# elrodrigues/deneva-plus

Measured on AMD Instinct MI355X. Metric: committed txns/sec (node) YCSB zipf0.9 at 1/2/4/8 GPUs; abort-set bit-exact, higher is better.
Workload: dtype u64; 1 GPU; YCSB config D: 16,777,216 rows/partition, 1,048,576-txn epoch in total; cc_alg=NO_WAIT, rows_per_partition=16777216, txns_per_epoch=1048576, txns_per_epoch_per_gpu=1048576, req_per_query=10, parallelism=1 GPU, decision_lanes=4, sequence_order=one origin

## Files before the change

### deneva-plus_amd/csrc/dvcc_kernels.hip

```cpp
#include <hip/hip_ext.h>

#include "dvcc_common.h"
#include "dvcc_tpcc.h"

#ifndef DVCC_PROBE_HIST_WAVES
#define DVCC_PROBE_HIST_WAVES 6
#endif

namespace dvcc {


constexpr int kPV = 4;
template <bool HIST, bool RSV>
__device__ __forceinline__ void probe_body(const Tables &tabs, const uint64_t *__restrict__ keys,
                                           const uint32_t *__restrict__ keys32,
                                                  const uint8_t *__restrict__ types,
                                                  const uint32_t *__restrict__ acc_txn,
                                                  const uint8_t *__restrict__ tables, uint64_t n,
                                                  uint32_t n_txn, uint32_t slog,
                                                  uint64_t *__restrict__ pairs,
                                                  uint32_t *__restrict__ tb_start,
                                                  uint32_t *__restrict__ tb_end,
                                                  uint8_t *__restrict__ tlen,
                                                  uint32_t *__restrict__ acc_row, Counters *ctr,
// ... 334 lines not shown
                pairs[a0 + pos] = pair_pack(row, t, (pos >> slog) ? 0u : pos, wr);
            }
        }
    }
    if (bad) set_err(ctr, ERRB_TXN);
    if (big_seen) set_err(ctr, ERRB_BIG);
    if (ts_bad) set_err(ctr, ERRB_TS);
}

void launch_probe_tb(hipStream_t s, const Tables &tabs, const uint64_t *keys, const uint8_t *types,
                     const uint32_t *recs, const uint32_t *txn_begin, uint64_t n_acc, uint32_t n_txn, uint32_t K,
                     uint32_t slog, uint64_t *pairs, uint8_t *tlen, uint32_t *acc_row, Counters *ctr,
                     const uint64_t *ts, hipEvent_t ev0, hipEvent_t ev1, const uint32_t *n_acc_dev) {
#ifndef DVCC_PROBE_TB_GRID
#define DVCC_PROBE_TB_GRID 4096
#endif
    uint32_t g = (n_txn + kBlock - 1) / kBlock;
    g = g < 1 ? 1 : (g > DVCC_PROBE_TB_GRID ? DVCC_PROBE_TB_GRID : g);
    DV_LAUNCH_EV(k_probe_tb, g, kBlock, 0, s, ev0, ev1, tabs, keys, types, recs, txn_begin, n_acc, n_txn, K, slog,
                 pairs, tlen, acc_row, ctr, ts, n_acc_dev);
}


__device__ __forceinline__ uint64_t sort_n(uint64_t n, const uint32_t *n_dev) {
    return n_dev && (uint64_t)*n_dev < n ? (uint64_t)*n_dev : n;
}

__device__ __forceinline__ uint32_t row_hash(uint64_t key, uint32_t hmul, int hbits) {
    return ((uint32_t)(key >> 32) * hmul) & ((1u << hbits) - 1u);
}
template <int W>
__device__ __forceinline__ uint32_t key_digit(uint64_t key, int shift, uint32_t hmul, int hbits) {
    return hmul ? row_hash(key, hmul, hbits) >> (hbits - W) : (uint32_t)(key >> shift) & ((1u << W) - 1u);
}

__global__ __launch_bounds__(kBlock) void k_radix_hist(const uint64_t *__restrict__ in, uint64_t n,
                                                       int shift, uint32_t *__restrict__ counts,
                                                       uint32_t nblocks, const uint32_t *__restrict__ n_dev,
                                                       uint32_t hmul, int hbits) {
    __shared__ uint32_t wc[4][kRadix];
    n = sort_n(n, n_dev);
    if ((uint64_t)blockIdx.x * kTile >= n) return;
    const uint32_t tid = threadIdx.x, lane = tid & 63, wave = tid >> 6;
    for (uint32_t d = tid; d < 4 * kRadix; d += kBlock) (&wc[0][0])[d] = 0;
    __syncthreads();
    const uint64_t base = (uint64_t)blockIdx.x * kTile + wave * (64 * kIPT);
    uint64_t k[kIPT];
#pragma unroll
    for (int j = 0; j < kIPT; j++) {
        const uint64_t idx = base + j * 64 + lane;
        k[j] = idx < n ? in[idx] : 0;
    }
#pragma unroll
    for (int j = 0; j < kIPT; j++) {
        const uint64_t idx = base + j * 64 + lane;
        const bool valid = idx < n;
        const uint32_t d = key_digit<kRadixBits>(k[j], shift, hmul, hbits);
        const uint32_t d0 = __builtin_amdgcn_readfirstlane(d);
        const uint64_t vmask = __ballot(valid);
        if (__ballot(valid && d == d0) == vmask) {
            if (lane == 0) wc[wave][d0] += (uint32_t)__popcll(vmask);
        } else if (valid) {
            atomicAdd(&wc[wave][d], 1u);
        }
    }
    __syncthreads();
    for (uint32_t d = tid; d < kRadix; d += kBlock)
        counts[(uint64_t)d * nblocks + blockIdx.x] = wc[0][d] + wc[1][d] + wc[2][d] + wc[3][d];
}

__global__ __launch_bounds__(kBlock) void k_radix_scan(uint32_t *__restrict__ counts, uint32_t nblocks,
                                                       uint32_t *__restrict__ digit_tot,
                                                       const uint32_t *__restrict__ n_dev) {
    __shared__ uint32_t lds4[4];
    uint32_t *c = counts + (uint64_t)blockIdx.x * nblocks;
    if (n_dev && nblocks_for(*n_dev) < nblocks) nblocks = nblocks_for(*n_dev);
    const uint32_t tot = block_chunk_scan256(c, nblocks, lds4);
    if (threadIdx.x == 0) digit_tot[blockIdx.x] = tot;
}

__global__ __launch_bounds__(kBlock) void k_radix_scatter(
    const uint64_t *__restrict__ in, uint64_t *__restrict__ out, uint64_t n, int shift, const uint32_t *__restrict__ counts,
    const uint32_t *__restrict__ digit_tot, uint32_t nblocks, const uint32_t *__restrict__ n_dev,
    uint32_t hmul, int hbits) {
    __shared__ __attribute__((aligned(16))) uint64_t skeys[kTile];
    n = sort_n(n, n_dev);
    if ((uint64_t)blockIdx.x * kTile >= n) return;
    __shared__ uint32_t wc[4][kRadix];
    __shared__ uint32_t dstart[kRadix];
    __shared__ uint64_t gbase[kRadix];
    __shared__ uint32_t lds4[4];
    const uint32_t tid = threadIdx.x, lane = tid & 63, wave = tid >> 6;
    const uint64_t tile0 = (uint64_t)blockIdx.x * kTile;

    {
        const uint32_t d = tid;
        const uint32_t dex = block_excl_scan256(digit_tot[d], lds4, nullptr);
        gbase[d] = (uint64_t)dex + counts[(uint64_t)d * nblocks + blockIdx.x];
        for (int w = 0; w < 4; w++) wc[w][d] = 0;
    }
    __syncthreads();

    const uint64_t base = tile0 + wave * (64 * kIPT);
    uint64_t k[kIPT];
    uint32_t r[kIPT];
#pragma unroll
    for (int j = 0; j < kIPT; j++) {
        const uint64_t idx = base + j * 64 + lane;
        k[j] = idx < n ? in[idx] : 0;
    }
#pragma unroll
    for (int j = 0; j < kIPT; j++) {
        const uint64_t idx = base + j * 64 + lane;
        const bool valid = idx < n;
        const uint32_t d = key_digit<kRadixBits>(k[j], shift, hmul, hbits);
        const uint64_t vmask = __ballot(valid);
        const uint64_t peers = match_digit(d, vmask);
        const uint32_t before = wc[wave][d];
        r[j] = before + mask_rank(peers);
        if (valid && lane == (uint32_t)__builtin_ctzll(peers)) wc[wave][d] = before + (uint32_t)__popcll(peers);
    }
    __syncthreads();
    {
        const uint32_t d = tid;
        const uint32_t c0 = wc[0][d], c1 = wc[1][d], c2 = wc[2][d], c3 = wc[3][d];
        wc[0][d] = 0;
        wc[1][d] = c0;
        wc[2][d] = c0 + c1;
        wc[3][d] = c0 + c1 + c2;
        const uint32_t ds = block_excl_scan256(c0 + c1 + c2 + c3, lds4, nullptr);
        dstart[d] = ds;
        gbase[d] -= ds;
    }
    __syncthreads();
#pragma unroll
    for (int j = 0; j < kIPT; j++) {
        const uint64_t idx = base + j * 64 + lane;
        if (idx < n) {
            const uint32_t d = key_digit<kRadixBits>(k[j], shift, hmul, hbits);
            const uint32_t pos = dstart[d] + wc[wave][d] + r[j];
            skeys[pos] = k[j];
        }
    }
    __syncthreads();
    const uint32_t tile_n = (uint32_t)((n - tile0) < (uint64_t)kTile ? (n - tile0) : kTile);
    for (uint32_t p = tid; p < tile_n; p += kBlock) {
        const uint64_t key = skeys[p];
        const uint32_t d = key_digit<kRadixBits>(key, shift, hmul, hbits);
        const uint64_t dst = gbase[d] + p;
        out[dst] = key;
    }
}

template <int W>
__global__ __launch_bounds__(kBlock) void k_radix_hist_w(const uint64_t *__restrict__ in, uint64_t n, int shift,
                                                         uint32_t *__restrict__ counts, uint32_t nblocks,
                                                         const uint32_t *__restrict__ n_dev, uint32_t hmul,
                                                         int hbits) {
    constexpr uint32_t R = 1u << W;
    __shared__ uint32_t wc[4][R];
    n = sort_n(n, n_dev);
    if ((uint64_t)blockIdx.x * kTile >= n) return;
    const uint32_t tid = threadIdx.x, lane = tid & 63, wave = tid >> 6;
    for (uint32_t d = tid; d < 4 * R; d += kBlock) (&wc[0][0])[d] = 0;
    __syncthreads();
    const uint64_t base = (uint64_t)blockIdx.x * kTile + wave * (64 * kIPT);
    uint64_t k[kIPT];
#pragma unroll
    for (int j = 0; j < kIPT; j++) {
        const uint64_t idx = base + j * 64 + lane;
        k[j] = idx < n ? in[idx] : 0;
    }
#pragma unroll
    for (int j = 0; j < kIPT; j++) {
        const uint64_t idx = base + j * 64 + lane;
        const bool valid = idx < n;
        const uint32_t d = key_digit<W>(k[j], shift, hmul, hbits);
        const uint32_t d0 = __builtin_amdgcn_readfirstlane(d);
        const uint64_t vmask = __ballot(valid);
        if (__ballot(valid && d == d0) == vmask) {
            if (lane == 0) wc[wave][d0] += (uint32_t)__popcll(vmask);
        } else if (valid) {
            atomicAdd(&wc[wave][d], 1u);
        }
    }
    __syncthreads();
    for (uint32_t d = tid; d < R; d += kBlock)
        counts[(uint64_t)d * nblocks + blockIdx.x] = wc[0][d] + wc[1][d] + wc[2][d] + wc[3][d];
}

template <int W>
__global__ __launch_bounds__(kBlock) void k_radix_scatter_w(const uint64_t *__restrict__ in, uint64_t *__restrict__ out,
                                                            uint64_t n, int shift, const uint32_t *__restrict__ counts,
                                                            const uint32_t *__restrict__ digit_tot, uint32_t nblocks,
                                                            const uint32_t *__restrict__ n_dev, uint32_t hmul,
                                                            int hbits) {
    constexpr uint32_t R = 1u << W, PER = R / kBlock;
    __shared__ __attribute__((aligned(16))) uint64_t skeys[kTile];
    __shared__ uint32_t wc[4][R];
    __shared__ uint32_t dstart[R];
    __shared__ uint32_t gbase[R];
    __shared__ uint32_t lds4[4];
    n = sort_n(n, n_dev);
    if ((uint64_t)blockIdx.x * kTile >= n) return;
    const uint32_t tid = threadIdx.x, lane = tid & 63, wave = tid >> 6;
    const uint64_t tile0 = (uint64_t)blockIdx.x * kTile;
    {
        uint32_t t[PER], sum = 0;
#pragma unroll
        for (uint32_t q = 0; q < PER; q++) {
            t[q] = digit_tot[tid * PER + q];
            sum += t[q];
        }
        uint32_t pre = block_excl_scan256(sum, lds4, nullptr);
#pragma unroll
        for (uint32_t q = 0; q < PER; q++) {
            const uint32_t d = tid * PER + q;
            gbase[d] = pre + counts[(uint64_t)d * nblocks + blockIdx.x];
            pre += t[q];
            wc[0][d] = wc[1][d] = wc[2][d] = wc[3][d] = 0;
        }
    }
    __syncthreads();
    const uint64_t base = tile0 + wave * (64 * kIPT);
    uint64_t k[kIPT];
    uint32_t r[kIPT];
#pragma unroll
    for (int j = 0; j < kIPT; j++) {
        const uint64_t idx = base + j * 64 + lane;
        k[j] = idx < n ? in[idx] : 0;
    }
#pragma unroll
    for (int j = 0; j < kIPT; j++) {
        const uint64_t idx = base + j * 64 + lane;
        const bool valid = idx < n;
        const uint32_t d = key_digit<W>(k[j], shift, hmul, hbits);
        uint64_t peers = __ballot(valid);
#pragma unroll
        for (int b = 0; b < W; b++) {
            const uint32_t bit = (d >> b) & 1u;
            const uint64_t m = __ballot(bit);
            peers &= bit ? m : ~m;
        }
        const uint32_t before = wc[wave][d];
        r[j] = before + mask_rank(peers);
        if (valid && lane == (uint32_t)__builtin_ctzll(peers)) wc[wave][d] = before + (uint32_t)__popcll(peers);
    }
    __syncthreads();
    {
        uint32_t tot[PER], sum = 0;
#pragma unroll
        for (uint32_t q = 0; q < PER; q++) {
            const uint32_t d = tid * PER + q;
            const uint32_t c0 = wc[0][d], c1 = wc[1][d], c2 = wc[2][d], c3 = wc[3][d];
            wc[0][d] = 0;
            wc[1][d] = c0;
            wc[2][d] = c0 + c1;
            wc[3][d] = c0 + c1 + c2;
            tot[q] = c0 + c1 + c2 + c3;
            sum += tot[q];
        }
        uint32_t ds = block_excl_scan256(sum, lds4, nullptr);
#pragma unroll
        for (uint32_t q = 0; q < PER; q++) {
            const uint32_t d = tid * PER + q;
            dstart[d] = ds;
            gbase[d] -= ds;
            ds += tot[q];
        }
    }
    __syncthreads();
#pragma unroll
    for (int j = 0; j < kIPT; j++) {
        const uint64_t idx = base + j * 64 + lane;
        if (idx < n) {
            const uint32_t d = key_digit<W>(k[j], shift, hmul, hbits);
            skeys[dstart[d] + wc[wave][d] + r[j]] = k[j];
        }
    }
    __syncthreads();
    const uint32_t tile_n = (uint32_t)((n - tile0) < (uint64_t)kTile ? (n - tile0) : kTile);
    for (uint32_t p = tid; p < tile_n; p += kBlock) {
        const uint64_t key = skeys[p];
        const uint32_t d = key_digit<W>(key, shift, hmul, hbits);
        out[(uint64_t)gbase[d] + p] = key;
    }
}

template <int W>
void wide_pass(hipStream_t s, const uint64_t *in, uint64_t *out, uint64_t n, int shift, uint32_t *counts,
               uint32_t *digit_tot, uint32_t nb, const uint32_t *n_dev, hipEvent_t e0, hipEvent_t e1,
               uint32_t hmul = 0, int hbits = 0) {
    DV_LAUNCH((k_radix_hist_w<W>), nb, kBlock, 0, s, in, n, shift, counts, nb, n_dev, hmul, hbits);
    DV_LAUNCH(k_radix_scan, 1u << W, kBlock, 0, s, counts, nb, digit_tot, n_dev);
    DV_LAUNCH_EV((k_radix_scatter_w<W>), nb, kBlock, 0, s, e0, e1, in, out, n, shift,
                          (const uint32_t *)counts, (const uint32_t *)digit_tot, nb, n_dev, hmul, hbits);
}

constexpr int kBucketThreads = 1024;
constexpr int kBucketWaves = kBucketThreads / 64;
constexpr int kBucketIdxBits = 32 - kBucketHiMax;
constexpr uint32_t kBucketCap = 1u << kBucketIdxBits;
constexpr int kBucketSteps = (int)kBucketCap / kBucketThreads;
static_assert((2 * kBucketCap + (kBucketWaves + 2) * kRadix + kBucketWaves) * sizeof(uint32_t) <= 160u * 1024u,
              "k_bucket_sort's LDS exceeds gfx950's 160 KiB per workgroup");

__device__ __forceinline__ uint32_t bucket_rank(uint32_t d, bool valid, uint32_t *wcw, uint32_t lane) {
    const uint64_t peers = match_digit(d, __ballot(valid));
    const uint32_t before = wcw[d];
    if (valid && lane == (uint32_t)__builtin_ctzll(peers)) wcw[d] = before + (uint32_t)__popcll(peers);
    return before + mask_rank(peers);
}

__device__ __forceinline__ void bucket_bases(uint32_t (*wc)[kRadix], uint32_t *tot, uint32_t *run) {
    const uint32_t tid = threadIdx.x, lane = tid & 63;
    uint32_t sum = 0;
    if (tid < (uint32_t)kRadix) {
#pragma unroll
        for (int w = 0; w < kBucketWaves; w++) {
            const uint32_t c = wc[w][tid];
            wc[w][tid] = sum;
            sum += c;
        }
        if (!run) tot[tid] = sum;
    }
    __syncthreads();
    if (!run && tid < 64) {
        uint32_t v[4], s4 = 0;
#pragma unroll
        for (int q = 0; q < 4; q++) {
            v[q] = tot[4 * lane + q];
            s4 += v[q];
        }
        uint32_t pre = wave_incl_sum(s4, lane) - s4;
#pragma unroll
        for (int q = 0; q < 4; q++) {
            tot[4 * lane + q] = pre;
            pre += v[q];
        }
    }
    if (!run) __syncthreads();
    if (tid < (uint32_t)kRadix) {
        const uint32_t b = run ? run[tid] : tot[tid];
        if (run) run[tid] = b + sum;
#pragma unroll
        for (int w = 0; w < kBucketWaves; w++) wc[w][tid] += b;
    }
    __syncthreads();
}

#ifdef DVCC_BUCKET_STAMPS
__device__ unsigned long long g_bucket_stamps[1024 * 4];
__device__ unsigned long long g_bucket_launch[4];
__device__ unsigned long long g_bucket_lmax;
struct BucketStamp {
    uint64_t t0;
    __device__ BucketStamp() : t0(wall_clock64()) {}
    __device__ void done(uint32_t b, uint32_t m) {
        __syncthreads();
        if (threadIdx.x != 0) return;
        const unsigned long long dt = wall_clock64() - t0;
        unsigned long long *w = g_bucket_stamps + (size_t)b * 4;
        atomicAdd(w + 0, 1ull);
        atomicAdd(w + 1, dt);
        atomicAdd(w + 2, (unsigned long long)m);
        atomicMax(w + 3, dt);
        atomicMax(&g_bucket_lmax, (dt << 20) | m);
        __threadfence();
        if (atomicAdd(&g_bucket_launch[3], 1ull) == (unsigned long long)gridDim.x - 1) {
            __threadfence();
            const unsigned long long mx = atomicExch(&g_bucket_lmax, 0ull);
            atomicAdd(&g_bucket_launch[0], 1ull);
            atomicAdd(&g_bucket_launch[1], mx >> 20);
            atomicAdd(&g_bucket_launch[2], mx & 0xFFFFFull);
            g_bucket_launch[3] = 0;
        }
    }
};
extern "C" int dv_debug_bucket_stamps(uint64_t *out, uint64_t *launch) {
    if (!out || !launch) return DV_ERR_ARG;
    if (hipDeviceSynchronize() != hipSuccess) return DV_ERR_HIP;
    if (hipMemcpyFromSymbol(out, HIP_SYMBOL(g_bucket_stamps), 1024 * 4 * 8) != hipSuccess) return DV_ERR_HIP;
    if (hipMemcpyFromSymbol(launch, HIP_SYMBOL(g_bucket_launch), 4 * 8) != hipSuccess) return DV_ERR_HIP;
    static const unsigned long long zero[1024 * 4] = {};
    if (hipMemcpyToSymbol(HIP_SYMBOL(g_bucket_stamps), zero, sizeof(zero)) != hipSuccess) return DV_ERR_HIP;
    if (hipMemcpyToSymbol(HIP_SYMBOL(g_bucket_launch), zero, 4 * 8) != hipSuccess) return DV_ERR_HIP;
    return DV_OK;
}
#endif

__global__ __launch_bounds__(kBucketThreads) void k_bucket_sort(uint64_t *__restrict__ in, uint64_t *__restrict__ out,
                                                                const uint32_t *__restrict__ digit_tot,
                                                                uint32_t hmul, int hbits, int hi_bits) {
#ifdef DVCC_BUCKET_STAMPS
    BucketStamp stamp_;
    struct StampAtExit {
        BucketStamp &s;
        uint32_t b, m;
        __device__ ~StampAtExit() { s.done(b, m); }
    } stamp_exit_{stamp_, blockIdx.x, 0u};
#endif
    __shared__ uint32_t tg[2][kBucketCap];
    __shared__ uint32_t wc[kBucketWaves][kRadix];
    __shared__ uint32_t tot[kRadix], run[kRadix];
    __shared__ uint32_t s_part[kBucketWaves];
    const uint32_t tid = threadIdx.x, lane = tid & 63, wave = tid >> 6, b = blockIdx.x;
    {
        uint32_t v = tid < b ? digit_tot[tid] : 0u;
#pragma unroll
        for (int off = 32; off > 0; off >>= 1) v += __shfl_xor(v, off, 64);
        if (lane == 0) s_part[wave] = v;
    }
    __syncthreads();
    uint32_t base = 0;
#pragma unroll
    for (int w = 0; w < kBucketWaves; w++) base += s_part[w];
    const uint32_t m = digit_tot[b];
#ifdef DVCC_BUCKET_STAMPS
    stamp_exit_.m = m;
#endif
    if (m <= 1) {
        if (m == 1 && tid == 0) out[base] = in[base];
        return;
    }
    const int passes = (hi_bits + kRadixBits - 1) / kRadixBits;
    const uint32_t hmask = (1u << hi_bits) - 1u;
    if (m <= kBucketCap) {
        {
            uint64_t kv[kBucketSteps];
#pragma unroll
            for (int s = 0; s < kBucketSteps; s++) {
                const uint32_t i = s * kBucketThreads + tid;
                kv[s] = i < m ? in[base + i] : 0ull;
            }
#pragma unroll
            for (int s = 0; s < kBucketSteps; s++) {
                const uint32_t i = s * kBucketThreads + tid;
                if (i < m) tg[0][i] = ((row_hash(kv[s], hmul, hbits) & hmask) << kBucketIdxBits) | i;
            }
        }
        __syncthreads();
        const uint32_t steps = (m + kBucketThreads - 1) / kBucketThreads;
        int cur = 0;
        for (int p = 0; p < passes; p++) {
            const int sh = kBucketIdxBits + kRadixBits * p;
            for (uint32_t d = lane; d < (uint32_t)kRadix; d += 64) wc[wave][d] = 0;
            uint32_t t[kBucketSteps], r[kBucketSteps];
#pragma unroll
            for (int s = 0; s < kBucketSteps; s++) {
                if ((uint32_t)s < steps) {
                    const uint32_t e = (wave * steps + s) * 64 + lane;
                    const bool valid = e < m;
                    t[s] = valid ? tg[cur][e] : 0u;
                    r[s] = bucket_rank((t[s] >> sh) & (kRadix - 1), valid, wc[wave], lane);
                }
            }
            __syncthreads();
            bucket_bases(wc, tot, nullptr);
#pragma unroll
            for (int s = 0; s < kBucketSteps; s++) {
                if ((uint32_t)s < steps) {
                    const uint32_t e = (wave * steps + s) * 64 + lane;
                    if (e < m) tg[cur ^ 1][wc[wave][(t[s] >> sh) & (kRadix - 1)] + r[s]] = t[s];
                }
            }
            __syncthreads();
            cur ^= 1;
        }
        uint64_t kv[kBucketSteps];
#pragma unroll
        for (int s = 0; s < kBucketSteps; s++) {
            const uint32_t i = s * kBucketThreads + tid;
            kv[s] = i < m ? in[base + (tg[cur][i] & (kBucketCap - 1))] : 0ull;
        }
#pragma unroll
        for (int s = 0; s < kBucketSteps; s++) {
            const uint32_t i = s * kBucketThreads + tid;
            if (i < m) out[base + i] = kv[s];
        }
        return;
    }
    uint64_t *A = in + base, *B = out + base;
    for (int p = 0; p < passes; p++) {
        const uint64_t *src = (p & 1) ? B : A;
        uint64_t *dst = (p & 1) ? A : B;
        const int sh = kRadixBits * p;
        if (tid < (uint32_t)kRadix) tot[tid] = 0;
        __syncthreads();
        for (uint32_t i0 = 0; i0 < m; i0 += kBucketThreads) {
            const uint32_t i = i0 + tid;
            const bool valid = i < m;
            const uint32_t d = valid ? ((row_hash(src[i], hmul, hbits) & hmask) >> sh) & (kRadix - 1) : 0u;
            const uint32_t d0 = __builtin_amdgcn_readfirstlane(d);
            const uint64_t vm = __ballot(valid);
            if (__ballot(valid && d == d0) == vm) {
                if (lane == 0 && vm) atomicAdd(&tot[d0], (uint32_t)__popcll(vm));
            } else if (valid) {
                atomicAdd(&tot[d], 1u);
            }
        }
        __syncthreads();
        if (tid < 64) {
            uint32_t v[4], s4 = 0;
#pragma unroll
            for (int q = 0; q < 4; q++) {
                v[q] = tot[4 * lane + q];
                s4 += v[q];
            }
            uint32_t pre = wave_incl_sum(s4, lane) - s4;
#pragma unroll
            for (int q = 0; q < 4; q++) {
                run[4 * lane + q] = pre;
                pre += v[q];
            }
        }
        __syncthreads();
        for (uint32_t c0 = 0; c0 < m; c0 += kBucketCap) {
            const uint32_t mc = m - c0 < kBucketCap ? m - c0 : kBucketCap;
            const uint32_t steps = (mc + kBucketThreads - 1) / kBucketThreads;
            for (uint32_t d = lane; d < (uint32_t)kRadix; d += 64) wc[wave][d] = 0;
            uint64_t k[kBucketSteps];
            uint32_t r[kBucketSteps];
#pragma unroll
            for (int s = 0; s < kBucketSteps; s++) {
                if ((uint32_t)s < steps) {
                    const uint32_t e = (wave * steps + s) * 64 + lane;
                    const bool valid = e < mc;
                    k[s] = valid ? src[c0 + e] : 0ull;
                    r[s] = bucket_rank(((row_hash(k[s], hmul, hbits) & hmask) >> sh) & (kRadix - 1), valid,
                                       wc[wave], lane);
                }
            }
            __syncthreads();
            bucket_bases(wc, tot, run);
#pragma unroll
            for (int s = 0; s < kBucketSteps; s++) {
                if ((uint32_t)s < steps) {
                    const uint32_t e = (wave * steps + s) * 64 + lane;
                    if (e < mc) dst[wc[wave][((row_hash(k[s], hmul, hbits) & hmask) >> sh) & (kRadix - 1)] + r[s]] = k[s];
                }
            }
            __syncthreads();
        }
    }
    if (!(passes & 1)) {
        for (uint32_t i = tid; i < m; i += kBucketThreads) B[i] = A[i];
    }
}

int radix_sort_rows(hipStream_t s, uint64_t *pairs[2], uint64_t n, int key_bits, uint32_t *counts,
                    uint32_t *digit_tot, hipEvent_t *scatter_ev, bool hist0_done, const uint32_t *n_dev,
                    bool lsd_only) {
    if (n == 0) return 0;
    const uint32_t nb = nblocks_for(n);
    int cur = 0, pass = 0;
    if (!lsd_only && bucket_sort_applies(n, key_bits, hist0_done, n_dev != nullptr)) {
        const int lo = kBucketLoBits(key_bits);
        const uint32_t hmul = kRowHashMul;
        hipEvent_t e0 = scatter_ev ? scatter_ev[0] : nullptr, e1 = scatter_ev ? scatter_ev[1] : nullptr;
        if (lo == 9)
            wide_pass<9>(s, pairs[0], pairs[1], n, 32, counts, digit_tot, nb, n_dev, e0, e1, hmul, key_bits);
        else if (lo == 10)
            wide_pass<10>(s, pairs[0], pairs[1], n, 32, counts, digit_tot, nb, n_dev, e0, e1, hmul, key_bits);
        else {
            DV_LAUNCH(k_radix_hist, nb, kBlock, 0, s, pairs[0], n, 32, counts, nb, n_dev, hmul, key_bits);
            DV_LAUNCH(k_radix_scan, kRadix, kBlock, 0, s, counts, nb, digit_tot, n_dev);
            DV_LAUNCH_EV(k_radix_scatter, nb, kBlock, 0, s, e0, e1, (const uint64_t *)pairs[0], pairs[1], n, 32,
                         (const uint32_t *)counts, (const uint32_t *)digit_tot, nb, n_dev, hmul, key_bits);
        }
        DV_LAUNCH_EV(k_bucket_sort, 1u << lo, kBucketThreads, 0, s, scatter_ev ? scatter_ev[2] : nullptr,
                     scatter_ev ? scatter_ev[3] : nullptr, pairs[1], pairs[0], (const uint32_t *)digit_tot,
                     hmul, key_bits, key_bits - lo);
        return 0;
    }
    const int wbits = radix_digit_bits(key_bits, hist0_done);
    if (wbits > kRadixBits) {
        for (int bit = 0; bit < key_bits; bit += wbits, pass++) {
            hipEvent_t e0 = scatter_ev ? scatter_ev[2 * pass] : nullptr, e1 = scatter_ev ? scatter_ev[2 * pass + 1] : nullptr;
            if (wbits == 9)
                wide_pass<9>(s, pairs[cur], pairs[cur ^ 1], n, 32 + bit, counts, digit_tot, nb, n_dev, e0, e1);
            else
                wide_pass<10>(s, pairs[cur], pairs[cur ^ 1], n, 32 + bit, counts, digit_tot, nb, n_dev, e0, e1);
            cur ^= 1;
        }
        return cur;
    }
    for (int bit = 0; bit < key_bits; bit += kRadixBits, pass++) {
        const int shift = 32 + bit;
        if (pass > 0 || !hist0_done)
            DV_LAUNCH(k_radix_hist, nb, kBlock, 0, s, pairs[cur], n, shift, counts, nb, n_dev, 0u, 0);
        DV_LAUNCH(k_radix_scan, kRadix, kBlock, 0, s, counts, nb, digit_tot, n_dev);
        DV_LAUNCH_EV(k_radix_scatter, nb, kBlock, 0, s, scatter_ev ? scatter_ev[2 * pass] : nullptr,
                     scatter_ev ? scatter_ev[2 * pass + 1] : nullptr, (const uint64_t *)pairs[cur], pairs[cur ^ 1], n,
                     shift, (const uint32_t *)counts, (const uint32_t *)digit_tot, nb, n_dev, 0u, 0);
        cur ^= 1;
    }
    return cur;
}

__device__ __forceinline__ uint32_t prev_entry_wr(const uint64_t *__restrict__ pairs, uint64_t e) {
    const uint64_t pe = pairs[e];
    while (e > 0) {
        const uint64_t qq = pairs[e - 1];
        if (pair_row(qq) != pair_row(pe) || pair_txn(qq) != pair_txn(pe)) break;
        e--;
    }
    return (uint32_t)pairs[e] & 1u;
}

__global__ __launch_bounds__(kBlock) void k_seg_prepare(const uint64_t *__restrict__ pairs, uint64_t n,
                                                        int calvin,
                                                        const uint32_t *__restrict__ tb_start,
                                                        uint64_t *__restrict__ el, Counters *ctr) {
    const uint32_t lane = threadIdx.x & 63;
    const uint64_t per_block = (uint64_t)kBlock * kPV;
    const uint64_t stride = (uint64_t)gridDim.x * per_block;
    for (uint64_t b0 = (uint64_t)blockIdx.x * per_block; b0 < n; b0 += stride) {
        const uint64_t i0 = b0 + (uint64_t)threadIdx.x * kPV;
        uint64_t p[kPV];
        if (i0 + kPV <= n) {
            const ulonglong2 a0 = *reinterpret_cast<const ulonglong2 *>(pairs + i0);
            const ulonglong2 a1 = *reinterpret_cast<const ulonglong2 *>(pairs + i0 + 2);
            p[0] = a0.x; p[1] = a0.y; p[2] = a1.x; p[3] = a1.y;
        } else {
#pragma unroll
            for (int j = 0; j < kPV; j++) p[j] = i0 + j < n ? pairs[i0 + j] : ~0ull;
        }
        uint64_t q = __shfl_up(p[kPV - 1], 1, 64);
        if (lane == 0) q = i0 > 0 && i0 - 1 < n ? pairs[i0 - 1] : ~0ull;
        uint32_t acc[kPV];
#pragma unroll
        for (int j = 0; j < kPV; j++) acc[j] = i0 + j < n ? tb_start[pair_txn(p[j])] + pair_pos(p[j]) : 0u;
        uint64_t out[kPV];
        bool dup_err = false;
#pragma unroll
        for (int j = 0; j < kPV; j++) {
            const uint64_t i = i0 + j;
            const uint64_t pj = p[j];
            const uint64_t pq = j == 0 ? q : p[j - 1];
            const uint32_t wr = (uint32_t)pj & 1u;
            uint32_t head = 1, dup = 0, bnd = 1;
            if (i > 0 && pair_row(pq) == pair_row(pj)) {
                head = 0;
                dup = pair_txn(pq) == pair_txn(pj);
                if (calvin) {
                    uint32_t pwr = (uint32_t)pq & 1u;
                    if (i >= 2 && pair_txn(pairs[i - 2]) == pair_txn(pq) && pair_row(pairs[i - 2]) == pair_row(pq))
                        pwr = prev_entry_wr(pairs, i - 1);
                    bnd = dup ? 0u : ((wr | pwr) ? 1u : 0u);
                }
            }
            dup_err |= dup && i < n;
            out[j] = el_pack(pair_txn(pj), acc[j],
                             ((calvin && bnd) ? EL_BND : 0u) | (dup ? EL_DUP : 0u) | (head ? EL_HEAD : 0u) | wr);
        }
        if (dup_err) {
            if (calvin) ctr->calvin_dups = 1u;
            else set_err(ctr, ERRB_DUP);
        }
        if (i0 + kPV <= n) {
            *reinterpret_cast<ulonglong2 *>(el + i0) = ulonglong2{out[0], out[1]};
            *reinterpret_cast<ulonglong2 *>(el + i0 + 2) = ulonglong2{out[2], out[3]};
        } else {
            for (int j = 0; j < kPV; j++)
                if (i0 + j < n) el[i0 + j] = out[j];
        }
    }
}

void launch_seg_prepare(hipStream_t s, const uint64_t *pairs, uint64_t n, int calvin,
                        const uint32_t *tb_start, uint64_t *el, Counters *ctr) {
    if (n == 0) return;
    uint64_t blocks = (n + (uint64_t)kBlock * kPV - 1) / ((uint64_t)kBlock * kPV);
    if (blocks > 4096) blocks = 4096;
    DV_LAUNCH(k_seg_prepare, (uint32_t)blocks, kBlock, 0, s, pairs, n, calvin, tb_start, el, ctr);
}

// ... 482 lines not shown
```

### deneva-plus_amd/csrc/dvcc_runtime.hip

```cpp
#include <hip/hip_runtime.h>

#include <algorithm>
#include <atomic>
#include <chrono>
#include <condition_variable>
#include <memory>
#include <mutex>
#include <cstdio>
#include <cstring>
#include <cstdlib>
#include <map>
#include <new>
#include <string>
#include <vector>

#include "dvcc_common.h"
#include "dvcc_tpcc.h"

using namespace dvcc;

namespace {

struct LaneOrder {
    std::mutex mu;
// ... 563 lines not shown
void dv_close(dv_ctx *c) {
    if (!c) return;
    if (c->stream) (void)hipStreamSynchronize(c->stream);
    for (auto &g : c->graphs)
        if (g.exec) (void)hipGraphExecDestroy(g.exec);
    c->graphs.clear();
    comm_free(c->comm);
    c->comm = nullptr;
    if (c->table_owner) {
        if (c->table_owner->lanes_open) c->table_owner->lanes_open--;
        for (auto &t : c->tab) t.ix = nullptr, t.bstart = nullptr, t.hbits = nullptr;
        c->f0 = c->pkey = nullptr;
        c->ktag = nullptr;
    }
    dfree(c->d_gate);
    if (c->lane_ev) (void)hipEventDestroy(c->lane_ev);
    for (auto &t : c->tab) {
        dfree(t.ix);
        dfree(t.bstart);
        dfree(t.hbits);
    }
    void *bufs[] = {c->f0, c->pkey, c->ktag, c->pairs[0], c->pairs[1], c->el, c->ew, c->counts,
                    c->digit_tot, c->rel[0], c->rel[1], c->vb8, c->tlen, c->acc_row,
                    c->ulist[0], c->ulist[1], c->tb_start, c->tb_end, c->desc, c->tile_ctr,
                    c->abounds, c->tword, c->carry_b, c->carry_tot, c->trk_part, c->bo_ws,
                    c->status, c->verdict, c->ctr, c->d_acc, c->d_keys, c->d_types,
                    c->d_tables, c->d_commit, c->d_txn, c->d_grant, c->d_tb, c->split_err,
                    c->d_args, c->d_oid, c->tp_dsnap,
                    c->row_state, c->b_status, c->b_tlen, c->b_map, c->kinfo, c->ktsum, c->kill_bits, c->gc_tb, c->gc_tot,
                    c->wire_ws, c->reply_bc,
                    c->hslot[0].acc, c->hslot[0].tb, c->hslot[1].acc, c->hslot[1].tb};
    for (void *b : bufs) dfree(b);
    for (auto &h : c->hslot) {
        if (h.copied) (void)hipEventDestroy(h.copied);
        if (h.drained) (void)hipEventDestroy(h.drained);
    }
    if (c->copy_stream) {
        (void)hipStreamSynchronize(c->copy_stream);
        (void)hipStreamDestroy(c->copy_stream);
    }
    if (c->h_ctr) (void)hipHostFree(c->h_ctr);
    if (c->h_pub) (void)hipHostFree(c->h_pub);
    if (c->wire_h) (void)hipHostFree(c->wire_h);
    if (c->wire_ev) (void)hipEventDestroy(c->wire_ev);
    for (auto &e : c->ev) if (e) (void)hipEventDestroy(e);
    for (auto &e : c->sev) if (e) (void)hipEventDestroy(e);
    for (auto &e : c->pev) if (e) (void)hipEventDestroy(e);
    for (auto &pr : c->kprof.pool) {
        (void)hipEventDestroy(pr.first);
        (void)hipEventDestroy(pr.second);
    }
    if (c->own_stream) (void)hipStreamDestroy(c->own_stream);
    if (c->lane_stream) (void)hipStreamDestroy(c->lane_stream);
    delete c;
}

int dv_open(dv_ctx **out, const dv_config *cfg) {
    if (!out || !cfg) return DV_ERR_ARG;
    *out = nullptr;
    if (cfg->cc_alg != DV_NO_WAIT && cfg->cc_alg != DV_WAIT_DIE && cfg->cc_alg != DV_OCC &&
        cfg->cc_alg != DV_CALVIN)
        return DV_ERR_ARG;
    if (cfg->workload != DV_YCSB && cfg->workload != DV_TPCC) return DV_ERR_ARG;
    if (cfg->max_txn == 0 || cfg->max_txn > kMaxTxn || cfg->max_acc == 0 ||
        cfg->max_acc > kMaxAcc || cfg->part_cnt == 0 || cfg->part_id >= cfg->part_cnt)
        return DV_ERR_ARG;
    int ndev = 0;
    if (dv_device_count(&ndev) != DV_OK || cfg->device < 0 || cfg->device >= ndev)
        return DV_ERR_NO_DEVICE;
    dv_ctx *c = new (std::nothrow) dv_ctx();
    if (!c) return DV_ERR_NOMEM;
    c->cfg = *cfg;
    c->cstride = cfg->workload == DV_TPCC ? 3u : 1u;
    int r = hip_fail(hipSetDevice(cfg->device), "hipSetDevice");
    if (!r) r = hip_fail(hipStreamCreateWithFlags(&c->own_stream, hipStreamNonBlocking), "stream");
    c->stream = c->own_stream;
    const uint64_t A = cfg->max_acc;
    const uint32_t T = cfg->max_txn;
    c->n_txn_cap_pad = (T + 3u) & ~3u;
    const uint32_t nb = nblocks_for(A);
    if (!r) r = dalloc(&c->pairs[0], A);
    if (!r) r = dalloc(&c->pairs[1], A);
    if (!r) r = dalloc(&c->counts, (uint64_t)kRadixMax * nb);
    if (!r) r = dalloc(&c->digit_tot, kRadixMax);
    if (!r) r = dalloc(&c->status, c->n_txn_cap_pad);
    if (!r) r = dalloc(&c->verdict, c->n_txn_cap_pad);
    if (!r) r = dalloc(&c->ctr, 1);
    const uint32_t rnb = (uint32_t)((A + kRTile - 1) / kRTile);
    if (!r) r = dalloc(&c->tb_start, c->n_txn_cap_pad);
    if (!r) r = dalloc(&c->tb_end, c->n_txn_cap_pad);
    if (!r) r = dalloc(&c->desc, rnb);
    if (!r) r = dalloc(&c->tile_ctr, kTileCtrs);
    if (!r) r = dalloc(&c->d_gate, 2);
    if (!r) r = hip_fail(hipEventCreateWithFlags(&c->lane_ev, hipEventDisableTiming), "hipEventCreate");
    if (!r) r = hip_fail(hipMemsetAsync(c->desc, 0, (size_t)rnb * 8, c->stream), "memset");
    if (!r) r = hip_fail(hipMemsetAsync(c->d_gate, 0, 2 * sizeof(uint32_t), c->stream), "memset");
    if (!r && cfg->cc_alg != DV_CALVIN) {
        r = dalloc(&c->rel[0], A);
        if (!r) r = dalloc(&c->rel[1], A);
        if (!r) r = dalloc(&c->tlen, c->n_txn_cap_pad);
        if (!r) r = dalloc(&c->acc_row, A);
        if (!r) r = dalloc(&c->ulist[0], T);
        if (!r) r = dalloc(&c->ulist[1], T);
        if (!r) r = dalloc(&c->abounds, kAsyncGroups);
        if (!r) r = dalloc(&c->tword, c->n_txn_cap_pad);
        if (!r) c->async_g = async_groups(cfg->device);
        int khz = 0;
        if (!r && hipDeviceGetAttribute(&khz, hipDeviceAttributeWallClockRate, cfg->device) == hipSuccess && khz > 0)
            c->wall_khz = (uint64_t)khz;
        c->async_idle_ticks = kAsyncIdleUs * c->wall_khz / 1000;
        c->vb8_cap = (uint64_t)c->n_txn_cap_pad << 4;
        if (!r) r = dalloc(&c->vb8, c->vb8_cap);
    }
    if (!r && cfg->cc_alg == DV_CALVIN) r = dalloc(&c->el, A);
    if (!r && cfg->cc_alg == DV_CALVIN) r = dalloc(&c->ew, A);
    constexpr size_t kMirBytes = ((sizeof(Counters) + 63) & ~size_t(63)) + 128;
    if (!r) r = hip_fail(hipHostMalloc(reinterpret_cast<void **>(&c->h_ctr), 2 * kMirBytes,
                                       hipHostMallocMapped | hipHostMallocCoherent),
                         "hipHostMalloc");
    if (!r) r = hip_fail(hipHostGetDevicePointer(reinterpret_cast<void **>(&c->d_hctr), c->h_ctr, 0),
                         "hipHostGetDevicePointer");
    if (!r) {
        std::memset(c->h_ctr, 0, 2 * kMirBytes);
        const size_t off = (sizeof(Counters) + 63) & ~size_t(63);
        for (int k = 0; k < 2; k++) {
            char *h = reinterpret_cast<char *>(c->h_ctr) + k * kMirBytes;
            char *d = reinterpret_cast<char *>(c->d_hctr) + k * kMirBytes;
            c->h_mir[k] = reinterpret_cast<Counters *>(h);
            c->d_mir[k] = reinterpret_cast<Counters *>(d);
            c->h_mseq[k] = reinterpret_cast<unsigned long long *>(h + off);
            c->d_mseq[k] = reinterpret_cast<unsigned long long *>(d + off);
        }
        c->h_cseq = c->h_mseq[0];
        c->d_cseq = c->d_mseq[0];
    }
    if (!r && cfg->cc_alg != DV_CALVIN) {
        r = hip_fail(hipHostMalloc(reinterpret_cast<void **>(&c->h_pub), sizeof(RoundPub),
                                   hipHostMallocMapped | hipHostMallocCoherent),
                     "hipHostMalloc");
        if (!r) r = hip_fail(hipHostGetDevicePointer(reinterpret_cast<void **>(&c->d_pub), c->h_pub, 0),
                             "hipHostGetDevicePointer");
        if (!r) std::memset(c->h_pub, 0, sizeof(RoundPub));
    }
    if (!r && ktiming(c)) {
        for (auto &e : c->ev) if (!r) r = hip_fail(hipEventCreate(&e), "hipEventCreate");
        for (auto &e : c->sev) if (!r) r = hip_fail(hipEventCreate(&e), "hipEventCreate");
        for (auto &e : c->pev) if (!r) r = hip_fail(hipEventCreate(&e), "hipEventCreate");
    }
    if (!r) r = hip_fail(hipMemsetAsync(c->verdict, 0, c->n_txn_cap_pad, c->stream), "memset");
    if (!r) r = hip_fail(hipStreamSynchronize(c->stream), "sync");
    if (r) {
        dv_close(c);
        return r;
    }
    *out = c;
    return DV_OK;
}

int dv_open_lane(dv_ctx *owner, dv_ctx **out) {
    if (!owner || !out) return DV_ERR_ARG;
    *out = nullptr;
    if (owner->table_owner || owner->comm) return DV_ERR_ARG;
    if (owner->phase != 0) return DV_ERR_STATE;
    if (!ctx_has_tables(owner)) return DV_ERR_NO_TABLE;
    dv_ctx *c = nullptr;
    int r = dv_open(&c, &owner->cfg);
    if (r) return r;
// ... 2762 lines not shown
```

Baseline: 164.8 million committed txns/s.

## Shrink bucket sort LDS and threads for two workgroups per CU, precompute bucket bases

The bucket-sort kernel now ranks in place with a single LDS tag buffer instead of a double buffer. It defaults to 512 threads with a launch bound allowing two workgroups per CU, and walks keys in fixed groups to limit register pressure. Scatter block 0 writes the per-digit exclusive prefix into a new digit_pre array, so each bucket block no longer reduces digit_tot itself. Digit matching uses a ballot-based bucket_match, and bucket_bases uses a wave-level scan in place of a serial single-wave pass. The aim is more occupancy and less LDS and sync cost. The risk is that in-place scatter within a pass is only safe because every value is read into registers before the barrier.

Result: faster. 170.6 million committed txns/s, median of 6 (+3.5%).

```diff
diff --git a/deneva-plus_amd/csrc/dvcc_kernels.hip b/deneva-plus_amd/csrc/dvcc_kernels.hip
--- a/deneva-plus_amd/csrc/dvcc_kernels.hip
+++ b/deneva-plus_amd/csrc/dvcc_kernels.hip
@@ -440,7 +440,7 @@
 __global__ __launch_bounds__(kBlock) void k_radix_scatter(
     const uint64_t *__restrict__ in, uint64_t *__restrict__ out, uint64_t n, int shift, const uint32_t *__restrict__ counts,
     const uint32_t *__restrict__ digit_tot, uint32_t nblocks, const uint32_t *__restrict__ n_dev,
-    uint32_t hmul, int hbits) {
+    uint32_t hmul, int hbits, uint32_t *__restrict__ digit_pre) {
     __shared__ __attribute__((aligned(16))) uint64_t skeys[kTile];
     n = sort_n(n, n_dev);
     if ((uint64_t)blockIdx.x * kTile >= n) return;
@@ -454,6 +454,7 @@
     {
         const uint32_t d = tid;
         const uint32_t dex = block_excl_scan256(digit_tot[d], lds4, nullptr);
+        if (digit_pre && blockIdx.x == 0) digit_pre[d] = dex;
         gbase[d] = (uint64_t)dex + counts[(uint64_t)d * nblocks + blockIdx.x];
         for (int w = 0; w < 4; w++) wc[w][d] = 0;
     }
@@ -552,7 +553,7 @@
                                                             uint64_t n, int shift, const uint32_t *__restrict__ counts,
                                                             const uint32_t *__restrict__ digit_tot, uint32_t nblocks,
                                                             const uint32_t *__restrict__ n_dev, uint32_t hmul,
-                                                            int hbits) {
+                                                            int hbits, uint32_t *__restrict__ digit_pre) {
     constexpr uint32_t R = 1u << W, PER = R / kBlock;
     __shared__ __attribute__((aligned(16))) uint64_t skeys[kTile];
     __shared__ uint32_t wc[4][R];
@@ -574,6 +575,7 @@
 #pragma unroll
         for (uint32_t q = 0; q < PER; q++) {
             const uint32_t d = tid * PER + q;
+            if (digit_pre && blockIdx.x == 0) digit_pre[d] = pre;
             gbase[d] = pre + counts[(uint64_t)d * nblocks + blockIdx.x];
             pre += t[q];
             wc[0][d] = wc[1][d] = wc[2][d] = wc[3][d] = 0;
@@ -648,90 +650,122 @@
 template <int W>
 void wide_pass(hipStream_t s, const uint64_t *in, uint64_t *out, uint64_t n, int shift, uint32_t *counts,
                uint32_t *digit_tot, uint32_t nb, const uint32_t *n_dev, hipEvent_t e0, hipEvent_t e1,
-               uint32_t hmul = 0, int hbits = 0) {
+               uint32_t hmul = 0, int hbits = 0, uint32_t *digit_pre = nullptr) {
     DV_LAUNCH((k_radix_hist_w<W>), nb, kBlock, 0, s, in, n, shift, counts, nb, n_dev, hmul, hbits);
     DV_LAUNCH(k_radix_scan, 1u << W, kBlock, 0, s, counts, nb, digit_tot, n_dev);
     DV_LAUNCH_EV((k_radix_scatter_w<W>), nb, kBlock, 0, s, e0, e1, in, out, n, shift,
-                          (const uint32_t *)counts, (const uint32_t *)digit_tot, nb, n_dev, hmul, hbits);
-}
-
-constexpr int kBucketThreads = 1024;
+                          (const uint32_t *)counts, (const uint32_t *)digit_tot, nb, n_dev, hmul, hbits, digit_pre);
+}
+
+#ifndef DVCC_BUCKET_THREADS
+#define DVCC_BUCKET_THREADS 512
+#endif
+constexpr int kBucketThreads = DVCC_BUCKET_THREADS;
+static_assert(kBucketThreads == 256 || kBucketThreads == 512 || kBucketThreads == 1024, "DVCC_BUCKET_THREADS");
 constexpr int kBucketWaves = kBucketThreads / 64;
 constexpr int kBucketIdxBits = 32 - kBucketHiMax;
 constexpr uint32_t kBucketCap = 1u << kBucketIdxBits;
 constexpr int kBucketSteps = (int)kBucketCap / kBucketThreads;
-static_assert((2 * kBucketCap + (kBucketWaves + 2) * kRadix + kBucketWaves) * sizeof(uint32_t) <= 160u * 1024u,
-              "k_bucket_sort's LDS exceeds gfx950's 160 KiB per workgroup");
+constexpr int kBucketGroup = 16;
+static_assert(kBucketSteps % kBucketGroup == 0, "k_bucket_sort walks its keys in whole groups of steps");
+constexpr uint32_t kBucketLds = (kBucketCap + (kBucketWaves + 2) * kRadix) * sizeof(uint32_t);
+constexpr int kBucketPerCu = kBucketThreads <= 512 ? 2 : 1;
+static_assert(kBucketPerCu * kBucketLds <= 160u * 1024u, "k_bucket_sort's workgroups exceed gfx950's 160 KiB of LDS per CU");
+constexpr int kBucketWavesPerSimd = kBucketPerCu * kBucketWaves / 4;
+
+__device__ __forceinline__ uint64_t bucket_match(uint32_t d, uint64_t valid) {
+    uint32_t lo = (uint32_t)valid, hi = (uint32_t)(valid >> 32);
+#pragma unroll
+    for (int b = 0; b < kRadixBits; b++) {
+        const uint32_t g = (uint32_t)((int32_t)(d << (31 - b)) >> 31);
+        const uint64_t m = __ballot((d & (1u << b)) != 0u);
+        lo &= ~((uint32_t)m ^ g);
+        hi &= ~((uint32_t)(m >> 32) ^ g);
+    }
+    return ((uint64_t)hi << 32) | lo;
+}
 
 __device__ __forceinline__ uint32_t bucket_rank(uint32_t d, bool valid, uint32_t *wcw, uint32_t lane) {
-    const uint64_t peers = match_digit(d, __ballot(valid));
+    const uint64_t peers = bucket_match(d, __ballot(valid));
     const uint32_t before = wcw[d];
     if (valid && lane == (uint32_t)__builtin_ctzll(peers)) wcw[d] = before + (uint32_t)__popcll(peers);
     return before + mask_rank(peers);
 }
 
 __device__ __forceinline__ void bucket_bases(uint32_t (*wc)[kRadix], uint32_t *tot, uint32_t *run) {
-    const uint32_t tid = threadIdx.x, lane = tid & 63;
-    uint32_t sum = 0;
-    if (tid < (uint32_t)kRadix) {
+    const uint32_t tid = threadIdx.x, lane = tid & 63, wave = tid >> 6;
+    const bool mine = tid < (uint32_t)kRadix;
+    uint32_t c[kBucketWaves], sum = 0, b = 0;
+    if (mine) {
+#pragma unroll
+        for (int w = 0; w < kBucketWaves; w++) c[w] = wc[w][tid];
 #pragma unroll
         for (int w = 0; w < kBucketWaves; w++) {
-            const uint32_t c = wc[w][tid];
-            wc[w][tid] = sum;
-            sum += c;
-        }
-        if (!run) tot[tid] = sum;
-    }
-    __syncthreads();
-    if (!run && tid < 64) {
-        uint32_t v[4], s4 = 0;
-#pragma unroll
-        for (int q = 0; q < 4; q++) {
-            v[q] = tot[4 * lane + q];
-            s4 += v[q];
-        }
-        uint32_t pre = wave_incl_sum(s4, lane) - s4;
-#pragma unroll
-        for (int q = 0; q < 4; q++) {
-            tot[4 * lane + q] = pre;
-            pre += v[q];
-        }
-    }
-    if (!run) __syncthreads();
-    if (tid < (uint32_t)kRadix) {
-        const uint32_t b = run ? run[tid] : tot[tid];
-        if (run) run[tid] = b + sum;
-#pragma unroll
-        for (int w = 0; w < kBucketWaves; w++) wc[w][tid] += b;
+            const uint32_t v = c[w];
+            c[w] = sum;
+            sum += v;
+        }
+        if (run) {
+            b = run[tid];
+            run[tid] = b + sum;
+        } else {
+            b = wave_incl_sum(sum, lane);
+            if (lane == 63) tot[wave] = b;
+            b -= sum;
+        }
+    }
+    if (!run) {
+        __syncthreads();
+        if (mine) {
+#pragma unroll
+            for (uint32_t w = 0; w < (uint32_t)kRadix / 64 - 1; w++) b += w < wave ? tot[w] : 0u;
+        }
+    }
+    if (mine) {
+#pragma unroll
+        for (int w = 0; w < kBucketWaves; w++) wc[w][tid] = c[w] + b;
     }
     __syncthreads();
 }
 
 #ifdef DVCC_BUCKET_STAMPS
+constexpr int kStampSlots = 8;
 __device__ unsigned long long g_bucket_stamps[1024 * 4];
 __device__ unsigned long long g_bucket_launch[4];
-__device__ unsigned long long g_bucket_lmax;
+__device__ unsigned long long g_bucket_ctx[kStampSlots * 8];
 struct BucketStamp {
     uint64_t t0;
     __device__ BucketStamp() : t0(wall_clock64()) {}
-    __device__ void done(uint32_t b, uint32_t m) {
+    __device__ void done(uint32_t b, uint32_t m, const void *ctx_key) {
         __syncthreads();
         if (threadIdx.x != 0) return;
-        const unsigned long long dt = wall_clock64() - t0;
+        const unsigned long long t1 = wall_clock64(), dt = t1 - t0;
         unsigned long long *w = g_bucket_stamps + (size_t)b * 4;
         atomicAdd(w + 0, 1ull);
         atomicAdd(w + 1, dt);
         atomicAdd(w + 2, (unsigned long long)m);
         atomicMax(w + 3, dt);
-        atomicMax(&g_bucket_lmax, (dt << 20) | m);
+        unsigned long long *c = nullptr;
+        for (int i = 0; i < kStampSlots && !c; i++) {
+            const unsigned long long k = atomicCAS(&g_bucket_ctx[i * 8 + 7], 0ull, (unsigned long long)ctx_key);
+            if (k == 0ull || k == (unsigned long long)ctx_key) c = g_bucket_ctx + i * 8;
+        }
+        if (!c) return;
+        atomicMax(c + 4, (dt << 20) | m);
+        atomicMax(c + 5, ~t0);
+        atomicMax(c + 6, t1);
         __threadfence();
-        if (atomicAdd(&g_bucket_launch[3], 1ull) == (unsigned long long)gridDim.x - 1) {
+        if (atomicAdd(c + 3, 1ull) == (unsigned long long)gridDim.x - 1) {
             __threadfence();
-            const unsigned long long mx = atomicExch(&g_bucket_lmax, 0ull);
+            const unsigned long long mx = atomicExch(c + 4, 0ull);
+            const unsigned long long first = ~atomicExch(c + 5, 0ull), last = atomicExch(c + 6, 0ull);
             atomicAdd(&g_bucket_launch[0], 1ull);
             atomicAdd(&g_bucket_launch[1], mx >> 20);
             atomicAdd(&g_bucket_launch[2], mx & 0xFFFFFull);
-            g_bucket_launch[3] = 0;
+            c[0] += 1;
+            c[1] += last - first;
+            if (last - first > c[2]) c[2] = last - first;
+            c[3] = 0;
         }
     }
 };
@@ -740,40 +774,32 @@
     if (hipDeviceSynchronize() != hipSuccess) return DV_ERR_HIP;
     if (hipMemcpyFromSymbol(out, HIP_SYMBOL(g_bucket_stamps), 1024 * 4 * 8) != hipSuccess) return DV_ERR_HIP;
     if (hipMemcpyFromSymbol(launch, HIP_SYMBOL(g_bucket_launch), 4 * 8) != hipSuccess) return DV_ERR_HIP;
+    if (hipMemcpyFromSymbol(launch + 4, HIP_SYMBOL(g_bucket_ctx), kStampSlots * 8 * 8) != hipSuccess) return DV_ERR_HIP;
     static const unsigned long long zero[1024 * 4] = {};
     if (hipMemcpyToSymbol(HIP_SYMBOL(g_bucket_stamps), zero, sizeof(zero)) != hipSuccess) return DV_ERR_HIP;
     if (hipMemcpyToSymbol(HIP_SYMBOL(g_bucket_launch), zero, 4 * 8) != hipSuccess) return DV_ERR_HIP;
+    if (hipMemcpyToSymbol(HIP_SYMBOL(g_bucket_ctx), zero, kStampSlots * 8 * 8) != hipSuccess) return DV_ERR_HIP;
     return DV_OK;
 }
 #endif
 
-__global__ __launch_bounds__(kBucketThreads) void k_bucket_sort(uint64_t *__restrict__ in, uint64_t *__restrict__ out,
-                                                                const uint32_t *__restrict__ digit_tot,
-                                                                uint32_t hmul, int hbits, int hi_bits) {
+__global__ __launch_bounds__(kBucketThreads, kBucketWavesPerSimd) void k_bucket_sort(
+    uint64_t *__restrict__ in, uint64_t *__restrict__ out, const uint32_t *__restrict__ digit_tot,
+    const uint32_t *__restrict__ digit_pre, uint32_t hmul, int hbits, int hi_bits) {
 #ifdef DVCC_BUCKET_STAMPS
     BucketStamp stamp_;
     struct StampAtExit {
         BucketStamp &s;
         uint32_t b, m;
-        __device__ ~StampAtExit() { s.done(b, m); }
-    } stamp_exit_{stamp_, blockIdx.x, 0u};
+        const void *key;
+        __device__ ~StampAtExit() { s.done(b, m, key); }
+    } stamp_exit_{stamp_, blockIdx.x, 0u, digit_tot};
 #endif
-    __shared__ uint32_t tg[2][kBucketCap];
+    __shared__ uint32_t tg[kBucketCap];
     __shared__ uint32_t wc[kBucketWaves][kRadix];
     __shared__ uint32_t tot[kRadix], run[kRadix];
-    __shared__ uint32_t s_part[kBucketWaves];
     const uint32_t tid = threadIdx.x, lane = tid & 63, wave = tid >> 6, b = blockIdx.x;
-    {
-        uint32_t v = tid < b ? digit_tot[tid] : 0u;
-#pragma unroll
-        for (int off = 32; off > 0; off >>= 1) v += __shfl_xor(v, off, 64);
-        if (lane == 0) s_part[wave] = v;
-    }
-    __syncthreads();
-    uint32_t base = 0;
-#pragma unroll
-    for (int w = 0; w < kBucketWaves; w++) base += s_part[w];
-    const uint32_t m = digit_tot[b];
+    const uint32_t m = digit_tot[b], base = digit_pre[b];
 #ifdef DVCC_BUCKET_STAMPS
     stamp_exit_.m = m;
 #endif
@@ -784,22 +810,22 @@
     const int passes = (hi_bits + kRadixBits - 1) / kRadixBits;
     const uint32_t hmask = (1u << hi_bits) - 1u;
     if (m <= kBucketCap) {
-        {
-            uint64_t kv[kBucketSteps];
-#pragma unroll
-            for (int s = 0; s < kBucketSteps; s++) {
-                const uint32_t i = s * kBucketThreads + tid;
+#pragma unroll 1
+        for (uint32_t g0 = 0; g0 < m; g0 += kBucketGroup * kBucketThreads) {
+            uint64_t kv[kBucketGroup];
+#pragma unroll
+            for (int s = 0; s < kBucketGroup; s++) {
+                const uint32_t i = g0 + s * kBucketThreads + tid;
                 kv[s] = i < m ? in[base + i] : 0ull;
             }
 #pragma unroll
-            for (int s = 0; s < kBucketSteps; s++) {
-                const uint32_t i = s * kBucketThreads + tid;
-                if (i < m) tg[0][i] = ((row_hash(kv[s], hmul, hbits) & hmask) << kBucketIdxBits) | i;
+            for (int s = 0; s < kBucketGroup; s++) {
+                const uint32_t i = g0 + s * kBucketThreads + tid;
+                if (i < m) tg[i] = ((row_hash(kv[s], hmul, hbits) & hmask) << kBucketIdxBits) | i;
             }
         }
         __syncthreads();
         const uint32_t steps = (m + kBucketThreads - 1) / kBucketThreads;
-        int cur = 0;
         for (int p = 0; p < passes; p++) {
             const int sh = kBucketIdxBits + kRadixBits * p;
             for (uint32_t d = lane; d < (uint32_t)kRadix; d += 64) wc[wave][d] = 0;
@@ -809,7 +835,7 @@
                 if ((uint32_t)s < steps) {
                     const uint32_t e = (wave * steps + s) * 64 + lane;
                     const bool valid = e < m;
-                    t[s] = valid ? tg[cur][e] : 0u;
+                    t[s] = valid ? tg[e] : 0u;
                     r[s] = bucket_rank((t[s] >> sh) & (kRadix - 1), valid, wc[wave], lane);
                 }
             }
@@ -819,25 +845,28 @@
             for (int s = 0; s < kBucketSteps; s++) {
                 if ((uint32_t)s < steps) {
                     const uint32_t e = (wave * steps + s) * 64 + lane;
-                    if (e < m) tg[cur ^ 1][wc[wave][(t[s] >> sh) & (kRadix - 1)] + r[s]] = t[s];
+                    if (e < m) tg[wc[wave][(t[s] >> sh) & (kRadix - 1)] + r[s]] = t[s];
                 }
             }
             __syncthreads();
-            cur ^= 1;
-        }
-        uint64_t kv[kBucketSteps];
-#pragma unroll
-        for (int s = 0; s < kBucketSteps; s++) {
-            const uint32_t i = s * kBucketThreads + tid;
-            kv[s] = i < m ? in[base + (tg[cur][i] & (kBucketCap - 1))] : 0ull;
-        }
-#pragma unroll
-        for (int s = 0; s < kBucketSteps; s++) {
-            const uint32_t i = s * kBucketThreads + tid;
-            if (i < m) out[base + i] = kv[s];
+        }
+#pragma unroll 1
+        for (uint32_t g0 = 0; g0 < m; g0 += kBucketGroup * kBucketThreads) {
+            uint64_t kv[kBucketGroup];
+#pragma unroll
+            for (int s = 0; s < kBucketGroup; s++) {
+                const uint32_t i = g0 + s * kBucketThreads + tid;
+                kv[s] = i < m ? in[base + (tg[i] & (kBucketCap - 1))] : 0ull;
+            }
+#pragma unroll
+            for (int s = 0; s < kBucketGroup; s++) {
+                const uint32_t i = g0 + s * kBucketThreads + tid;
+                if (i < m) out[base + i] = kv[s];
+            }
         }
         return;
     }
+    constexpr uint32_t kChunk = kBucketGroup * kBucketThreads;
     uint64_t *A = in + base, *B = out + base;
     for (int p = 0; p < passes; p++) {
         const uint64_t *src = (p & 1) ? B : A;
@@ -873,14 +902,14 @@
             }
         }
         __syncthreads();
-        for (uint32_t c0 = 0; c0 < m; c0 += kBucketCap) {
-            const uint32_t mc = m - c0 < kBucketCap ? m - c0 : kBucketCap;
+        for (uint32_t c0 = 0; c0 < m; c0 += kChunk) {
+            const uint32_t mc = m - c0 < kChunk ? m - c0 : kChunk;
             const uint32_t steps = (mc + kBucketThreads - 1) / kBucketThreads;
             for (uint32_t d = lane; d < (uint32_t)kRadix; d += 64) wc[wave][d] = 0;
-            uint64_t k[kBucketSteps];
-            uint32_t r[kBucketSteps];
-#pragma unroll
-            for (int s = 0; s < kBucketSteps; s++) {
+            uint64_t k[kBucketGroup];
+            uint32_t r[kBucketGroup];
+#pragma unroll
+            for (int s = 0; s < kBucketGroup; s++) {
                 if ((uint32_t)s < steps) {
                     const uint32_t e = (wave * steps + s) * 64 + lane;
                     const bool valid = e < mc;
@@ -892,7 +921,7 @@
             __syncthreads();
             bucket_bases(wc, tot, run);
 #pragma unroll
-            for (int s = 0; s < kBucketSteps; s++) {
+            for (int s = 0; s < kBucketGroup; s++) {
                 if ((uint32_t)s < steps) {
                     const uint32_t e = (wave * steps + s) * 64 + lane;
                     if (e < mc) dst[wc[wave][((row_hash(k[s], hmul, hbits) & hmask) >> sh) & (kRadix - 1)] + r[s]] = k[s];
@@ -915,20 +944,21 @@
     if (!lsd_only && bucket_sort_applies(n, key_bits, hist0_done, n_dev != nullptr)) {
         const int lo = kBucketLoBits(key_bits);
         const uint32_t hmul = kRowHashMul;
+        uint32_t *digit_pre = digit_tot + kRadixMax;
         hipEvent_t e0 = scatter_ev ? scatter_ev[0] : nullptr, e1 = scatter_ev ? scatter_ev[1] : nullptr;
         if (lo == 9)
-            wide_pass<9>(s, pairs[0], pairs[1], n, 32, counts, digit_tot, nb, n_dev, e0, e1, hmul, key_bits);
+            wide_pass<9>(s, pairs[0], pairs[1], n, 32, counts, digit_tot, nb, n_dev, e0, e1, hmul, key_bits, digit_pre);
         else if (lo == 10)
-            wide_pass<10>(s, pairs[0], pairs[1], n, 32, counts, digit_tot, nb, n_dev, e0, e1, hmul, key_bits);
+            wide_pass<10>(s, pairs[0], pairs[1], n, 32, counts, digit_tot, nb, n_dev, e0, e1, hmul, key_bits, digit_pre);
         else {
             DV_LAUNCH(k_radix_hist, nb, kBlock, 0, s, pairs[0], n, 32, counts, nb, n_dev, hmul, key_bits);
             DV_LAUNCH(k_radix_scan, kRadix, kBlock, 0, s, counts, nb, digit_tot, n_dev);
             DV_LAUNCH_EV(k_radix_scatter, nb, kBlock, 0, s, e0, e1, (const uint64_t *)pairs[0], pairs[1], n, 32,
-                         (const uint32_t *)counts, (const uint32_t *)digit_tot, nb, n_dev, hmul, key_bits);
+                         (const uint32_t *)counts, (const uint32_t *)digit_tot, nb, n_dev, hmul, key_bits, digit_pre);
         }
         DV_LAUNCH_EV(k_bucket_sort, 1u << lo, kBucketThreads, 0, s, scatter_ev ? scatter_ev[2] : nullptr,
                      scatter_ev ? scatter_ev[3] : nullptr, pairs[1], pairs[0], (const uint32_t *)digit_tot,
-                     hmul, key_bits, key_bits - lo);
+                     (const uint32_t *)digit_pre, hmul, key_bits, key_bits - lo);
         return 0;
     }
     const int wbits = radix_digit_bits(key_bits, hist0_done);
@@ -950,7 +980,7 @@
         DV_LAUNCH(k_radix_scan, kRadix, kBlock, 0, s, counts, nb, digit_tot, n_dev);
         DV_LAUNCH_EV(k_radix_scatter, nb, kBlock, 0, s, scatter_ev ? scatter_ev[2 * pass] : nullptr,
                      scatter_ev ? scatter_ev[2 * pass + 1] : nullptr, (const uint64_t *)pairs[cur], pairs[cur ^ 1], n,
-                     shift, (const uint32_t *)counts, (const uint32_t *)digit_tot, nb, n_dev, 0u, 0);
+                     shift, (const uint32_t *)counts, (const uint32_t *)digit_tot, nb, n_dev, 0u, 0, (uint32_t *)nullptr);
         cur ^= 1;
     }
     return cur;
diff --git a/deneva-plus_amd/csrc/dvcc_runtime.hip b/deneva-plus_amd/csrc/dvcc_runtime.hip
--- a/deneva-plus_amd/csrc/dvcc_runtime.hip
+++ b/deneva-plus_amd/csrc/dvcc_runtime.hip
@@ -669,7 +669,7 @@
     if (!r) r = dalloc(&c->pairs[0], A);
     if (!r) r = dalloc(&c->pairs[1], A);
     if (!r) r = dalloc(&c->counts, (uint64_t)kRadixMax * nb);
-    if (!r) r = dalloc(&c->digit_tot, kRadixMax);
+    if (!r) r = dalloc(&c->digit_tot, 2 * kRadixMax);
     if (!r) r = dalloc(&c->status, c->n_txn_cap_pad);
     if (!r) r = dalloc(&c->verdict, c->n_txn_cap_pad);
     if (!r) r = dalloc(&c->ctr, 1);
```
